# speedinghzl/DSRG

Hardware: AMD Instinct MI355X
Metric: images/sec DSRG train step (VGG16 321x321, 21-class) (higher is better)
Workload: dtype bf16 backbone (fp32 master weights) + f32/f64 supervision path

## Files before the change

dsrg_amd/_lib.py:

```python
import ctypes
import os

import torch

_HERE = os.path.dirname(os.path.abspath(__file__))
LIB_PATH = os.path.join(_HERE, os.environ.get("DSRG_LIB") or "libdsrg_hip.so")

OK, ERR_INVALID, ERR_HIP, ERR_UNSUPPORTED, ERR_NOMEM = 0, -1, -2, -3, -4


class DsrgError(RuntimeError):
    def __init__(self, code, msg):
        RuntimeError.__init__(self, "libdsrg_hip error %d: %s" % (code, msg))
        self.code = code


class CrfParams(ctypes.Structure):
    _fields_ = [("w_bilateral", ctypes.c_float), ("theta_alpha_x", ctypes.c_float),
                ("theta_alpha_y", ctypes.c_float), ("theta_beta_r", ctypes.c_float),
                ("theta_beta_g", ctypes.c_float), ("theta_beta_b", ctypes.c_float),
                ("w_gaussian", ctypes.c_float), ("theta_gamma_x", ctypes.c_float),
                ("theta_gamma_y", ctypes.c_float), ("n_iters", ctypes.c_int32)]

    @classmethod
# ... 46 lines not shown
    "dsrg_seed_loss_plain": (_i, [_i, _i, _i, _vp, _vp, _vp, _vp, _vp]),
    "dsrg_expand_loss": (_i, [_i, _i, _i, _vp, _vp, _d, _d, _vp, _vp, _vp, _vp]),
    "dsrg_confusion_matrix": (_i, [_sz, _vp, _vp, _i, _i, _vp, _vp]),
    "dsrg_multiscale_unary": (_i, [_i, _i, ctypes.POINTER(_vp), ctypes.POINTER(ctypes.c_int32), ctypes.POINTER(ctypes.c_int32), _i, _i,
                                   _f, _vp, _vp, _vp, _vp]),
    "dsrg_im2col3x3_nhwc16": (_i, [_vp, _vp, _i, _i, _i, _i, _i, _vp]),
    "dsrg_relu_bwd_bias_bf16": (_i, [_vp, _vp, _vp, _vp, _vp, _i, ctypes.c_long, _i, ctypes.c_float, _vp]),
    "dsrg_col2im3x3_nhwc_bf16": (_i, [_vp, _vp, _i, _i, _i, _i, _i, _vp]),
    "dsrg_avgpool3x3_s1_bf16": (_i, [_vp, _vp, _i, _i, _i, _i, _vp]),
    "dsrg_conv_igemm_backward_residual_bf16": (_i, [_vp] * 8 + [_i, _vp, _sz] + [_i] * 6 + [_vp]),
    "dsrg_pack_conv_weight_scaled_f32": (_i, [_vp, _vp, _vp, _vp, _i, _i, _i, _vp]),
    "dsrg_aspp_shift_sum_f32": (_i, [_vp, _vp, _vp, _vp] + [_i] * 6 + [_vp]),
    "dsrg_aspp_shift_gather_bf16": (_i, [_vp, _vp, _vp] + [_i] * 6 + [_vp]),
    "dsrg_defer_reductions": (_i, [_i]),
    "dsrg_flush_reductions": (_i, [_vp]),
    "dsrg_conv_igemm_residual_bf16": (_i, [_vp] * 6 + [_i] * 8 + [_vp]),
    "dsrg_conv_igemm_split_f32": (_i, [_vp, _vp, _vp, _vp] + [_i] * 8 + [_vp]),
    "dsrg_add_relu_bf16": (_i, [_vp, _vp, _vp, _sz, _vp]),
    "dsrg_relu_mask_bf16": (_i, [_vp, _vp, _vp, _vp, _sz, _vp]),
    "dsrg_bias_grad_bf16": (_i, [_vp, _vp, _vp, _i, ctypes.c_long, _i, _vp]),
    "dsrg_heads_forward_bf16": (_i, [_vp, _i, _vp, _vp, _vp, _i, _i, _i, _i, _vp]),
    "dsrg_conv3x3_direct_bf16": (_i, [_vp, _vp, _vp, _vp, _i, _i, _i, _i, _i, _i, _vp]),
    "dsrg_conv3x3_direct_dgrad_workspace": (_sz, [_i]),
    "dsrg_conv3x3_direct_dgrad_bf16": (_i, [_vp] * 6 + [_sz] + [_i] * 5 + [_vp]),
    "dsrg_conv_igemm_supported": (_i, [_i, _i, _i]),
    "dsrg_conv_igemm_bf16": (_i, [_vp, _vp, _vp, _vp, _vp, _i, _i, _i, _i, _i, _i, _i, _i, ctypes.c_float, ctypes.c_ulonglong, _vp, _sz,
                                  _vp]),
    "dsrg_conv_igemm_workspace": (_sz, []),
    "dsrg_conv_igemm_dgrad_workspace": (_sz, [_i] * 5),
    "dsrg_conv_igemm_dgrad_bf16": (_i, [_vp] * 6 + [_i] * 7 + [_f, _vp, _sz, _vp]),
# ... 51 lines not shown
```

dsrg_amd/csrc/backbone_ops.hip:

```cpp
#include "common.h"
#include <algorithm>
#include <cstring>

namespace dsrg {

__device__ __forceinline__ float bf16_lo(uint32_t w) { return __uint_as_float(w << 16); }
__device__ __forceinline__ float bf16_hi(uint32_t w) { return __uint_as_float(w & 0xffff0000u); }
__device__ __forceinline__ uint32_t f32_to_bf16_rne(float f) {
    uint32_t u = __float_as_uint(f);
    if ((u & 0x7fffffffu) > 0x7f800000u) return (u >> 16) | 0x40u;
    return (u + 0x7fffu + ((u >> 16) & 1u)) >> 16;
}
__device__ __forceinline__ uint32_t pack_bf16(float lo, float hi) { return f32_to_bf16_rne(lo) | (f32_to_bf16_rne(hi) << 16); }

constexpr int kRbThreads = 256;

__global__ __launch_bounds__(kRbThreads) void relu_bwd_bias_kernel(const uint4 *__restrict__ g, const uint4 *__restrict__ y,
                                                                    uint4 *__restrict__ gm, float *__restrict__ part,
                                                                    int rows, int C8, int rows_per_block, float scale) {
    __shared__ float red[kRbThreads][9];
    const int lanes_r = kRbThreads / C8;
    const int cg = threadIdx.x % C8, rl = threadIdx.x / C8;
    float acc[8] = {0.f, 0.f, 0.f, 0.f, 0.f, 0.f, 0.f, 0.f};
    if (rl < lanes_r) {
// ... 1066 lines not shown
    if (gw) {
        HeadArgs a;
        for (int k = 0; k < 4; k++) a.x[k] = static_cast<const uint16_t *>(x[k < nbr ? k : 0]);
        a.w = w; a.bias = nullptr; a.out = nullptr; a.nbr = nbr; a.M = M; a.K = K; a.O = O; a.HW = HW;
        const int nch = heads_bwd_chunks(M), rows = ((M + nch - 1) / nch + 1) & ~1;
        const size_t lds = (size_t)kDwRows2 * (K * 2 + 64) + 32 * kDwGPitch * sizeof(float);
        if (lds > 160 * 1024) {
            hipLaunchKernelGGL(heads_bwd_dw_kernel, dim3(nch, nbr), dim3(256), 0, stream, a, g, partial, rows);
        } else {
            static LdsGrant grant;
            if (int rc2 = ensure_dynamic_lds(reinterpret_cast<const void *>(&heads_bwd_dw_split_kernel), lds, grant)) return rc2;
            hipLaunchKernelGGL(heads_bwd_dw_split_kernel, dim3(nch, nbr), dim3(256), lds, stream, a, g, partial, rows);
        }
        DSRG_LAUNCH_CHECK();
        const size_t n = (size_t)nbr * O * K;
        hipLaunchKernelGGL(heads_bwd_dw_reduce_kernel, dim3((unsigned)((n + 255) / 256)), dim3(256), 0, stream, partial, gw, nch, n);
        DSRG_LAUNCH_CHECK();
    }
    return DSRG_OK;
}

}
```

dsrg_amd/csrc/common.h:

```cpp
#pragma once
#include <hip/hip_runtime.h>
#include <stdint.h>
#include <stddef.h>
#include <atomic>
#include "../../include/dsrg_hip.h"

namespace dsrg {

int set_error(int code, const char *fmt, ...);
#define DSRG_HIP_CHECK(expr)                                                              \
    do {                                                                                  \
        hipError_t _e = (expr);                                                           \
        if (_e != hipSuccess)                                                             \
            return ::dsrg::set_error(DSRG_ERR_HIP, "%s failed: %s (%s:%d)", #expr,        \
                                     hipGetErrorString(_e), __FILE__, __LINE__);          \
    } while (0)
#define DSRG_LAUNCH_CHECK() DSRG_HIP_CHECK(hipGetLastError())

__device__ __forceinline__ void colsum_block(const float *__restrict__ p, float *__restrict__ out, int rows, int cout, int bx, float (*red)[64]) {
    const int cl = threadIdx.x & 63, c = bx * 64 + cl, q = threadIdx.x >> 6;
    float s0 = 0.0f, s1 = 0.0f;
    int r = q;
    for (; r + 16 < rows; r += 32) {
        s0 += p[(size_t)r * cout + c];
// ... 23 lines not shown
            s2 += part[(size_t)(b + 16) * C + c];
            s3 += part[(size_t)(b + 24) * C + c];
        }
        for (; b < nblk; b += 8) s0 += part[(size_t)b * C + c];
    }
    if (on) red[sl][cl] = (s0 + s1) + (s2 + s3);
    __syncthreads();
    if (on && sl == 0 && c < C) {
        float s = 0.f;
#pragma unroll
        for (int k = 0; k < 8; ++k) s += red[k][cl];
        bias_grad[c] = s;
    }
}
bool defer_reduction(int kind, const float *part, float *out, int rows, int cols);

struct LdsGrant { std::atomic<size_t> bytes[16]; LdsGrant() { for (auto &b : bytes) b.store(0, std::memory_order_relaxed); } };
inline int ensure_dynamic_lds(const void *fn, size_t bytes, std::atomic<size_t> &granted) {
    size_t have = granted.load(std::memory_order_acquire);
    if (bytes <= have) return DSRG_OK;
    if (bytes > 64 * 1024) {
        hipError_t e = hipFuncSetAttribute(fn, hipFuncAttributeMaxDynamicSharedMemorySize, (int)bytes);
        if (e != hipSuccess)
            return set_error(DSRG_ERR_HIP, "cannot reserve %zu B of dynamic LDS: %s", bytes, hipGetErrorString(e));
    }
    while (have < bytes && !granted.compare_exchange_weak(have, bytes, std::memory_order_release, std::memory_order_acquire)) {}
    return DSRG_OK;
}
inline int ensure_dynamic_lds(const void *fn, size_t bytes, LdsGrant &g) {
    int dev = 0;
// ... 200 lines not shown
```

dsrg_amd/csrc/conv_direct.hip:

```cpp
#include "common.h"

namespace dsrg {
namespace {
typedef __attribute__((ext_vector_type(8))) __bf16 bf16x8;
typedef __attribute__((ext_vector_type(2))) __bf16 bf16x2;
typedef __attribute__((ext_vector_type(2))) float f32x2;
typedef __attribute__((ext_vector_type(16))) float f32x16;
typedef __attribute__((address_space(3))) void lds_void;
constexpr int kTH = 8, kTW = 16;
constexpr int kHH = kTH + 2, kHW = kTW + 2;

template <int CIN, int COUT, int TPW_ = (CIN == 64 ? 2 : 1)> struct Cfg {
    static constexpr int CG = CIN / 16;
    static constexpr int KS = 9 * CG;
    static constexpr int TPW = TPW_;
    static constexpr int WGS = TPW * KS * 4 <= 144 ? 2 : 1;
    static constexpr int NG = COUT / (32 * TPW);
    static constexpr int PG = 4 / NG;
    static constexpr int MT = 4 / PG;
    static constexpr int KPS = WGS == 2 ? 2 : 4;
    static constexpr int SPT = CG / KPS;
    static constexpr int STEPS = 9 * SPT;
    static constexpr bool DMA = CIN == 128 && COUT == 128;
    static constexpr int CPR = CIN / 8;
// ... 751 lines not shown
    a.B = B; a.H = H; a.W = W; a.cin = cin; a.roles = cin < 64 ? 1 : cin / 64;
    a.tiles_x = (W + kTW - 1) / kTW; a.tiles_y = (H + kTH - 1) / kTH;
    const long items = (long)B * a.tiles_x * a.tiles_y * a.roles;
    if (B < 1 || H < 1 || W < 1 || items > 0x7fffffffL) return set_error(DSRG_ERR_INVALID, "conv3x3_wgrad: bad shape");
    a.nitems = (int)items;
    const int grid = wgrad_grid(B, H, W, cin, cout);
    if (workspace_bytes < conv3x3_wgrad_workspace(B, H, W, cin, cout))
        return set_error(DSRG_ERR_INVALID, "conv3x3_wgrad: workspace of %zu bytes, %zu needed", workspace_bytes,
                         conv3x3_wgrad_workspace(B, H, W, cin, cout));
    if (cin == 3) {
        static LdsGrant grant;
        const size_t lds = 2 * kHH * kHW * kC3Pix + 3 * kTH * kTW * kC3Row;
        if (int rc = ensure_dynamic_lds(reinterpret_cast<const void *>(&conv3x3_c3_wgrad_kernel), lds, grant)) return rc;
        hipLaunchKernelGGL(conv3x3_c3_wgrad_kernel, dim3(grid), dim3(256), lds, stream, a);
        DSRG_LAUNCH_CHECK();
        if (out_f32) hipLaunchKernelGGL(conv3x3_c3_wgrad_reduce_kernel<true>, dim3(64), dim3(1024), 0, stream, workspace, gw, grid);
        else hipLaunchKernelGGL(conv3x3_c3_wgrad_reduce_kernel<false>, dim3(64), dim3(1024), 0, stream, workspace, gw, grid);
        DSRG_LAUNCH_CHECK();
        return DSRG_OK;
    }
    if (int rc = cout == 64 ? launch_wgrad_variant<2>(a, grid, stream) : launch_wgrad_variant<4>(a, grid, stream)) return rc;
    if (out_f32)
        hipLaunchKernelGGL(conv3x3_wgrad_reduce_kernel<true>, dim3(cout * 9 * cin / 64), dim3(1024), 0, stream, workspace, gw, grid, a.roles,
                           cout, cin);
    else
        hipLaunchKernelGGL(conv3x3_wgrad_reduce_kernel<false>, dim3(cout * 9 * cin / 64), dim3(1024), 0, stream, workspace, gw, grid, a.roles,
                           cout, cin);
    DSRG_LAUNCH_CHECK();
    return DSRG_OK;
}

bool conv3x3_direct_supported(int cin, int cout) {
    return ((cin == 64 || cin == 128) && (cout == 64 || cout == 128)) || (cin == 3 && cout == 64);
}

size_t conv3x3_direct_colsum_workspace(int cout) { return (size_t)2 * device_cus() * (size_t)cout * sizeof(float); }

int launch_conv3x3_direct(const void *x, const void *w, const float *bias, void *y, int B, int H, int W, int cin, int cout,
                          int relu, hipStream_t stream, const void *mask, float *colsum, void *colsum_ws, size_t colsum_ws_bytes) {
    if (!conv3x3_direct_supported(cin, cout))
        return set_error(DSRG_ERR_INVALID, "conv3x3_direct: %d -> %d channels is not one of 64/128 -> 64/128 or 3 -> 64", cin, cout);
    if ((mask || colsum) && (cin == 3 || !mask || !colsum))
        return set_error(DSRG_ERR_UNSUPPORTED, "conv3x3_direct: the masked form takes 64 / 128 channels, mask and bias gradient together");
    if (mask && (long long)B * H * W * cout * 2 >= 0x7fffffffLL)
// ... 30 lines not shown
```

dsrg_amd/csrc/conv_igemm.hip:

```cpp
#include "common.h"
#include <algorithm>
#include <cstdlib>
#include <cstring>
#include <functional>
#include <map>
#include <mutex>
#include <queue>
#include <vector>

namespace dsrg {
namespace {
typedef __attribute__((ext_vector_type(8))) __bf16 bf16x8;
typedef __attribute__((ext_vector_type(2))) __bf16 bf16x2;
typedef __attribute__((ext_vector_type(2))) float f32x2;
typedef __attribute__((ext_vector_type(16))) float f32x16;
typedef __attribute__((address_space(3))) void lds_void;

constexpr int kBM = 256, kBN = 256;
constexpr int kOutRow = 128 * 2 + 16;
constexpr int kOutWave = 64 * kOutRow;
constexpr uint32_t kOob = 0x80000000u;
constexpr int kRowTab = 8 * kOutWave;
constexpr int kRowTabBytes = kBM * 4;

// ... 1369 lines not shown
    const int ks_mix = wgrad_ksplit(M, tiles, 256, (double)ngroups * cout * k * k * cin * 4.0, true);
    if (ks_mix > ks) ks = ks_mix;
    if (ngroups == 1) ks = wgrad_ksplit_cap(M, ks);
    return (size_t)ngroups * ks * cout * k * k * cin * sizeof(float);
}

static int launch_wgrad_reduce(const IgemmWgradArgs &a, void *const *gw, int ngroups, int cin, int cout, int k, int out_bf16, hipStream_t stream) {
    WgradReduceArgs r;
    memset(&r, 0, sizeof(r));
    r.ksplit = a.ksplit;
    r.n4 = (size_t)cout * k * k * cin / 4;
    r.scale = t_wgrad_scale;
    r.per_o4 = (size_t)k * k * cin / 4;
    for (int q = 0; q < ngroups; q++) { r.part[q] = a.g[q].part; r.gw[q] = gw[q]; }
    const dim3 rgrid((unsigned)((r.n4 + 255) / 256), (unsigned)ngroups);
    if (out_bf16) hipLaunchKernelGGL(conv_igemm_wgrad_reduce_kernel<true>, rgrid, dim3(256), 0, stream, r);
    else hipLaunchKernelGGL(conv_igemm_wgrad_reduce_kernel<false>, rgrid, dim3(256), 0, stream, r);
    DSRG_LAUNCH_CHECK();
    return DSRG_OK;
}

int launch_conv_igemm_wgrad(const void *const *x, const void *const *g, void *const *gw, const int *dil, int ngroups, void *workspace,
                            size_t workspace_bytes, int B, int H, int W, int cin, int cout, int k, int out_bf16, hipStream_t stream) {
    if (ngroups < 1 || ngroups > 4) return set_error(DSRG_ERR_INVALID, "conv_igemm_wgrad: 1..4 groups");
    if (!conv_igemm_wgrad_launchable(cin, cout, k))
        return set_error(DSRG_ERR_UNSUPPORTED, "conv_igemm_wgrad: cin %% 64 == 0, cout %% 64 == 0, k in (1, 3) required (got %d, %d, %d)", cin, cout, k);
    const long long M = (long long)B * H * W;
    if (M <= 0 || M * cin * 2 >= 0x7fffffffLL || M * cout * 2 >= 0x7fffffffLL)
        return set_error(DSRG_ERR_UNSUPPORTED, "conv_igemm_wgrad: tensor too large for 32-bit buffer offsets");
    const size_t need = conv_igemm_wgrad_workspace(ngroups, B, H, W, cin, cout, k);
    if (!workspace || workspace_bytes < need) return set_error(DSRG_ERR_INVALID, "conv_igemm_wgrad: workspace of %zu bytes needed", need);
    IgemmWgradArgs a;
    memset(&a, 0, sizeof(a));
    a.ngroups = ngroups; a.B = B; a.H = H; a.W = W; a.Cin = cin; a.Cout = cout; a.taps = k * k; a.M = (int)M;
// ... 170 lines not shown
```

dsrg_amd/csrc/deferred.hip:

```cpp
#include "common.h"
#include <mutex>
#include <cstring>

namespace dsrg {
namespace {

constexpr int kMaxDeferred = 48;
struct DeferredReduction {
    const float *part;
    float *out;
    int rows, cols, kind, first_block;
};
struct DeferredArgs {
    DeferredReduction e[kMaxDeferred];
    int n;
};

__global__ __launch_bounds__(1024) void deferred_reductions_kernel(DeferredArgs a) {
    __shared__ float red_c[16][64];
    __shared__ float red_b[8][33];
    const int b = (int)blockIdx.x;
    int k = 0;
    while (k + 1 < a.n && b >= a.e[k + 1].first_block) k++;
    const DeferredReduction d = a.e[k];
    if (d.kind == 0) colsum_block(d.part, d.out, d.rows, d.cols, b - d.first_block, red_c);
    else bias_finalize_block(d.part, d.out, d.rows, d.cols, b - d.first_block, red_b);
}

std::mutex g_mutex;
bool g_on = false;
DeferredArgs g_list;
int g_blocks = 0;

}

bool defer_reduction(int kind, const float *part, float *out, int rows, int cols) {
    std::lock_guard<std::mutex> lock(g_mutex);
    if (!g_on || g_list.n >= kMaxDeferred || rows < 1 || cols < 1 || (kind == 0 && cols % 64)) return false;
    DeferredReduction &d = g_list.e[g_list.n++];
    d.part = part; d.out = out; d.rows = rows; d.cols = cols; d.kind = kind; d.first_block = g_blocks;
    g_blocks += kind == 0 ? cols / 64 : (cols + 31) / 32;
    return true;
}

int defer_reductions(int on) {
    std::lock_guard<std::mutex> lock(g_mutex);
    if (on && !g_on) { memset(&g_list, 0, sizeof(g_list)); g_blocks = 0; }
    g_on = on != 0;
    return DSRG_OK;
}

int flush_reductions(hipStream_t stream) {
    DeferredArgs a;
    int blocks;
    {
        std::lock_guard<std::mutex> lock(g_mutex);
        a = g_list;
        blocks = g_blocks;
        memset(&g_list, 0, sizeof(g_list));
        g_blocks = 0;
    }
    if (a.n == 0) return DSRG_OK;
    hipLaunchKernelGGL(deferred_reductions_kernel, dim3(blocks), dim3(1024), 0, stream, a);
    DSRG_LAUNCH_CHECK();
    return DSRG_OK;
}

}

extern "C" int dsrg_defer_reductions(int on) { return dsrg::defer_reductions(on); }
extern "C" int dsrg_flush_reductions(void *stream) { return dsrg::flush_reductions(static_cast<hipStream_t>(stream)); }
```

dsrg_amd/ops.py:

```python
import ctypes
import threading

import torch

from . import _lib
from ._lib import CrfParams, check


def _stream():
    return ctypes.c_void_p(torch.cuda.current_stream().cuda_stream)


def _ptr(t):
    return ctypes.c_void_p(t.data_ptr()) if t is not None else None


def _f32c(t, name):
    if not (t.is_cuda and t.dtype == torch.float32 and t.is_contiguous()):
        raise ValueError("%s must be a contiguous float32 CUDA tensor" % name)
    return t


_defer = [False]
_defer_keep = []


def _keep_until_flush(*tensors):
    if _defer[0]:
        _defer_keep.extend(t for t in tensors if t is not None)


@__import__("contextlib").contextmanager
def deferred_reductions(enabled=True):
    if not enabled or _defer[0]:
        yield
        return
    L = _lib.lib()
    check(L.dsrg_defer_reductions(1))
    _defer[0] = True
    try:
        yield
    finally:
        _defer[0] = False
        rc = L.dsrg_flush_reductions(_stream())
        L.dsrg_defer_reductions(0)
        del _defer_keep[:]
        check(rc)


class Context(object):

    def __init__(self, max_batch, C, H, W):
        _lib.require_gpu()
        self.max_batch, self.C, self.H, self.W = int(max_batch), int(C), int(H), int(W)
        self.device = torch.cuda.current_device()
        h = ctypes.c_void_p()
        check(_lib.lib().dsrg_ctx_create(self.max_batch, self.C, self.H, self.W, ctypes.byref(h)))
        self._h = h
# ... 597 lines not shown
    else:
        _check_kept_packs(weight, fwd, dg, pack)
    return fwd, (dg if want_dgrad else None)


def conv3x3_wgrad(x, g, out_dtype=torch.bfloat16, out=None):
    B, cin, H, W = x.shape
    cout = g.shape[1]
    cl = torch.channels_last
    if not (x.is_cuda and x.dtype == torch.bfloat16 and g.dtype == torch.bfloat16 and tuple(g.shape) == (B, cout, H, W)
            and (cin, cout) in WGRAD_CONV_SHAPES):
        raise ValueError("conv3x3_wgrad needs bf16 CUDA tensors with (cin, cout) in %s" % (WGRAD_CONV_SHAPES,))
    x = x if x.is_contiguous(memory_format=cl) else x.contiguous(memory_format=cl)
    g = g if g.is_contiguous(memory_format=cl) else g.contiguous(memory_format=cl)
    need = _lib.lib().dsrg_conv3x3_wgrad_workspace(B, H, W, cin, cout)
    key = (x.device.index, torch.cuda.current_stream().cuda_stream)
    ws = _wgrad_ws.get(key)
    if ws is None or ws.numel() < need:
        ws = _wgrad_ws[key] = torch.empty(need, dtype=torch.uint8, device=x.device)
    if out_dtype not in (torch.bfloat16, torch.float32):
        raise ValueError("conv3x3_wgrad: bf16 or float32 output")
    gw = _dest(out, (cout, cin, 3, 3), out_dtype, x.device, True)
    fn = _lib.lib().dsrg_conv3x3_wgrad_f32 if out_dtype == torch.float32 else _lib.lib().dsrg_conv3x3_wgrad_bf16
    check(fn(_ptr(x), _ptr(g), _ptr(gw), _ptr(ws), ws.numel(), B, H, W, cin, cout, _stream()))
    return gw


def conv_igemm_supported(cin, cout, k):
    return bool(_lib.lib().dsrg_conv_igemm_supported(int(cin), int(cout), int(k)))


def set_igemm_variant(v):
    _lib.lib().dsrg_debug_set_igemm_variant(int(v))


def pack_conv_weight(weight, for_dgrad=False, dtype=torch.bfloat16):
    k = weight.shape[2]
# ... 148 lines not shown

def conv_igemm_backward(g, packed_d, x, dilation, mask=None, mask_scale=1.0, ksize=3, gw_out=None, gb_out=None):
    B, cout, H, W = g.shape
    cin = x.shape[1]
    cl = torch.channels_last
    if not (g.is_cuda and g.dtype == torch.bfloat16 and x.dtype == torch.bfloat16 and tuple(x.shape) == (B, cin, H, W)
            and packed_d.dtype == torch.bfloat16 and tuple(packed_d.shape) == (cin, cout // 64, ksize * ksize, 64)
            and packed_d.is_contiguous() and x.is_contiguous(memory_format=cl)
            and (mask is None or (mask.dtype == torch.bfloat16 and tuple(mask.shape) == (B, cin, H, W) and mask.is_contiguous(memory_format=cl)))):
        raise ValueError("conv_igemm_backward needs bf16 channels_last g / x (/ mask) of one geometry and the data-gradient packing")
    g = g if g.is_contiguous(memory_format=cl) else g.contiguous(memory_format=cl)
    L = _lib.lib()
    need = L.dsrg_conv_igemm_wgrad_workspace(1, B, H, W, cin, cout, ksize)
    if need == 0:
        raise ValueError("conv_igemm_backward: 256 | cin (or cin = 128), 256 | cout required (got %d, %d)" % (cin, cout))
    key = (g.device.index, torch.cuda.current_stream().cuda_stream)
    ws = _igemm_ws.get(key)
    if ws is None or ws.numel() < need:
        ws = _igemm_ws[key] = torch.empty(need, dtype=torch.uint8, device=g.device)
    gx = torch.empty((B, cin, H, W), dtype=torch.bfloat16, device=g.device, memory_format=cl)
    gw = _dest(gw_out, (cout, cin, ksize, ksize), torch.float32, g.device, True)
    gb = cws = None
    if mask is not None:
        gb = _dest(gb_out, (cin,), torch.float32, g.device)
        cws = torch.empty(L.dsrg_conv_igemm_dgrad_workspace(1, B, H, W, cin), dtype=torch.uint8, device=g.device)
        _keep_until_flush(cws)
    check(L.dsrg_conv_igemm_backward_bf16(_ptr(g), _ptr(packed_d), _ptr(x), _ptr(mask), _ptr(gx), _ptr(gw), int(dilation), _ptr(gb),
                                          float(mask_scale), _ptr(cws), cws.numel() if cws is not None else 0, _ptr(ws), ws.numel(),
                                          B, H, W, cin, cout, ksize, _stream()))
    return gx, gw, gb


def conv_igemm_backward_residual(g, packed_d, x, dilation, ksize, mask=None, res=None, gw_scale=None, gw_out=None):
    B, cout, H, W = g.shape
    cin = x.shape[1]
    cl = torch.channels_last
    ok = lambda t: t.dtype == torch.bfloat16 and tuple(t.shape) == (B, cin, H, W) and t.is_contiguous(memory_format=cl)
    if not (g.is_cuda and g.dtype == torch.bfloat16 and ok(x) and packed_d.dtype == torch.bfloat16 and packed_d.is_contiguous()
            and tuple(packed_d.shape) == (cin, cout // 64, ksize * ksize, 64) and (mask is None or ok(mask)) and (res is None or ok(res))):
        raise ValueError("conv_igemm_backward_residual needs bf16 channels_last g / x (/ mask / res) of one geometry and the data-gradient packing")
    g = g if g.is_contiguous(memory_format=cl) else g.contiguous(memory_format=cl)
    L = _lib.lib()
    need = L.dsrg_conv_igemm_wgrad_workspace(1, B, H, W, cin, cout, ksize)
    if need == 0:
        raise ValueError("conv_igemm_backward_residual: 256 | cin (or cin = 128 with a 3x3 kernel), 256 | cout required (got %d, %d)" % (cin, cout))
    key = (g.device.index, torch.cuda.current_stream().cuda_stream)
    ws = _igemm_ws.get(key)
    if ws is None or ws.numel() < need:
        ws = _igemm_ws[key] = torch.empty(need, dtype=torch.uint8, device=g.device)
    gx = torch.empty((B, cin, H, W), dtype=torch.bfloat16, device=g.device, memory_format=cl)
    gw = _dest(gw_out, (cout, cin, ksize, ksize), torch.float32, g.device, True)
    sc = None if gw_scale is None else _f32c(gw_scale, "gw_scale")
    check(L.dsrg_conv_igemm_backward_residual_bf16(_ptr(g), _ptr(packed_d), _ptr(x), _ptr(mask), _ptr(res), _ptr(gx), _ptr(gw), _ptr(sc),
                                                   int(dilation), _ptr(ws), ws.numel(), B, H, W, cin, cout, ksize, _stream()))
    return gx, gw


_igemm_sk_ws = {}


def _igemm_sk_workspace(device):
    key = (device.index, torch.cuda.current_stream(device).cuda_stream)
    ws = _igemm_sk_ws.get(key)
    if ws is None:
        ws = _igemm_sk_ws[key] = torch.empty(_lib.lib().dsrg_conv_igemm_workspace(), dtype=torch.uint8, device=device)
    return ws

# ... 27 lines not shown
    B, cin, H, W = xs[0].shape
    cout = gs[0].shape[1]
    cl = torch.channels_last
    if not (1 <= n <= 4 and len(gs) == n and len(dilations) == n) or out_dtype not in (torch.float32, torch.bfloat16):
        raise ValueError("conv_igemm_wgrad: 1..4 groups, float32 or bfloat16 result")
    for x, g in zip(xs, gs):
        if not (x.is_cuda and x.dtype == torch.bfloat16 and g.dtype == torch.bfloat16 and tuple(x.shape) == (B, cin, H, W)
                and tuple(g.shape) == (B, cout, H, W)):
            raise ValueError("conv_igemm_wgrad needs bf16 CUDA tensors of one geometry")
    xs = [x if x.is_contiguous(memory_format=cl) else x.contiguous(memory_format=cl) for x in xs]
    gs = [g if g.is_contiguous(memory_format=cl) else g.contiguous(memory_format=cl) for g in gs]
    L = _lib.lib()
    need = L.dsrg_conv_igemm_wgrad_workspace(n, B, H, W, cin, cout, ksize)
    if need == 0:
        raise ValueError("conv_igemm_wgrad: 64 | cin, 64 | cout, k in (1, 3) required (got %d, %d, %d)" % (cin, cout, ksize))
    key = (xs[0].device.index, torch.cuda.current_stream().cuda_stream)
    ws = _igemm_ws.get(key)
    if ws is None or ws.numel() < need:
        ws = _igemm_ws[key] = torch.empty(need, dtype=torch.uint8, device=xs[0].device)
    gws = [_dest(outs[i] if outs is not None else None, (cout, cin, ksize, ksize), out_dtype, xs[0].device, True) for i in range(n)]
    vp = ctypes.c_void_p * n
    check(L.dsrg_conv_igemm_wgrad_bf16(vp(*[x.data_ptr() for x in xs]), vp(*[g.data_ptr() for g in gs]),
                                       vp(*[w.data_ptr() for w in gws]), (ctypes.c_int * n)(*[int(d) for d in dilations]), n,
                                       _ptr(ws), ws.numel(), B, H, W, cin, cout, ksize, int(out_dtype == torch.bfloat16), _stream()))
    return gws


def heads_forward(xs, weight, bias):
    B, K, H, W = xs[0].shape
    n, O = weight.shape[0], weight.shape[1]
    cl = torch.channels_last
    xs = [x if x.is_contiguous(memory_format=cl) else x.contiguous(memory_format=cl) for x in xs]
    if not all(x.is_cuda and x.dtype == torch.bfloat16 and x.shape == xs[0].shape for x in xs) or len(xs) != n:
        raise ValueError("heads_forward needs n bf16 CUDA activations of one shape")
    _f32c(weight, "weight")
# ... 6 lines not shown


def heads_backward(xs, weight, g, need_gx=True, relu_scale=0.0):
    B, K, H, W = xs[0].shape
    n, O = weight.shape[0], weight.shape[1]
    cl = torch.channels_last
    xs = [x if x.is_contiguous(memory_format=cl) else x.contiguous(memory_format=cl) for x in xs]
    _f32c(weight, "weight")
    g = g.contiguous()
    _f32c(g, "g")
    L = _lib.lib()
    M = B * H * W
    gx = torch.empty((n, B, H, W, K), dtype=torch.bfloat16, device=g.device) if need_gx else None
    gw = torch.empty((n, O, K), dtype=torch.float32, device=g.device)
    part = torch.empty(L.dsrg_heads_backward_chunks(M) * n * O * K, dtype=torch.float32, device=g.device)
    ptrs = (ctypes.c_void_p * 4)(*([x.data_ptr() for x in xs] + [None] * (4 - n)))
    if relu_scale > 0.0 and need_gx:
        gb = torch.empty((n, K), dtype=torch.float32, device=g.device)
        ws = torch.empty(L.dsrg_heads_backward_relu_workspace(n, M, K), dtype=torch.uint8, device=g.device)
        _keep_until_flush(ws)
        check(L.dsrg_heads_backward_relu_bf16(ptrs, n, _ptr(weight), _ptr(g), _ptr(gx), M * K * 2, _ptr(gw), _ptr(part),
                                              float(relu_scale), _ptr(gb), _ptr(ws), ws.numel(), B, H * W, K, O, _stream()))
        return [gx[k].permute(0, 3, 1, 2) for k in range(n)], gw, gb
    check(L.dsrg_heads_backward_bf16(ptrs, n, _ptr(weight), _ptr(g), _ptr(gx), M * K * 2, _ptr(gw), _ptr(part), B, H * W, K, O,
                                     _stream()))
    return ([gx[k].permute(0, 3, 1, 2) for k in range(n)] if need_gx else None), gw


def maxpool3x3_out_size(n, stride, ceil_mode):
    num = n + 2 - 3
    o = (-(-num // stride) if ceil_mode else num // stride) + 1
    if (o - 1) * stride >= n + 1:
        o -= 1
# ... 59 lines not shown
```

dsrg_amd/retrain.py:

```python
import torch
import torch.nn as nn
import torch.nn.functional as F

import os as _os

from .backbone import VGG16ASPP, GemmConv2d, _ConvFn, _bf16_run
from .trainer import CaffeSGD

_FUSE_RES = _os.environ.get("DSRG_RESNET_FUSE_RES", "1") == "1"


def interp_shrink(label, factor=8):
    H, W = label.shape[-2:]
    if (H - 1) % factor == 0 and (W - 1) % factor == 0:
        return label[..., ::factor, ::factor]
    h, w = (H - 1) // factor + 1, (W - 1) // factor + 1
    return F.interpolate(label.float(), size=(h, w), mode="bilinear", align_corners=True)


def seg_softmax_loss(logits, label, ignore_label=255):
    return F.cross_entropy(logits.float(), label.reshape(label.shape[0], *label.shape[-2:]).long(),
                           ignore_index=ignore_label, reduction="mean")


# ... 341 lines not shown
    def load(self, state_path):
        from .checkpoint import load_snapshot
        return load_snapshot(self, state_path)

    def step(self, images, label):
        if self.reducer is not None:
            self.reducer.prepare()
        else:
            self.opt.zero_grad()
        self.opt.base_lr = poly_lr(self.base_lr, self.opt.iter, self.max_iter)
        x = images.contiguous(memory_format=torch.channels_last) if self.device.type == "cuda" else images
        with torch.autocast(self.device.type, dtype=self.amp_dtype, enabled=self.amp_dtype is not None):
            logits = self.net(x)
        loss = seg_softmax_loss(logits, interp_shrink(label, 8))
        from .ops import deferred_reductions
        with deferred_reductions(self.defer_bias):
            loss.backward()
        if self.reducer is not None:
            self.reducer.finish()
        self.opt.step()
        return loss.detach()
```

dsrg_amd/trainer.py:

```python
import os

import torch

from .backbone import VGG16ASPP
from .ops import dsrg_supervision_loss


_SGD_PACK = os.environ.get("DSRG_SGD_PACK", "1") != "0"


class CaffeSGD(object):

    def __init__(self, groups, base_lr=5e-4, momentum=0.9, weight_decay=5e-4, gamma=0.33, stepsize=1000):
        self.groups = groups
        self.base_lr, self.momentum, self.wd, self.gamma, self.stepsize = base_lr, momentum, weight_decay, gamma, stepsize
        self.iter = 0
        for g in self.groups:
            g["bufs"] = [torch.zeros_like(p, memory_format=torch.preserve_format) for p in g["params"]]
            g["buf_lr"] = None
        if _SGD_PACK:
            from .ops import keep_weight_packs
            keep_weight_packs([p for g in self.groups for p in g["params"] if p.is_cuda], self)

    def lr(self):
# ... 155 lines not shown
        if self.overlap_build:
            from .ops import crf_prepare
            main = torch.cuda.current_stream()
            self.side.wait_stream(main)
            with torch.cuda.stream(self.side):
                crf_prepare(images, cues.shape[1], cues.shape[2], cues.shape[3])
        with torch.autocast(self.device.type, dtype=self.amp_dtype, enabled=self.amp_dtype is not None):
            logits = self.net(x)
        logits = logits.float().contiguous()
        if self.overlap_build:
            torch.cuda.current_stream().wait_stream(self.side)
            total, losses = self.loss_fn(logits, images, labels, cues, prepared=True)
        else:
            total, losses = self.loss_fn(logits, images, labels, cues)
        from .ops import deferred_reductions
        with deferred_reductions(self.defer_bias):
            total.backward()
        if self.reducer is not None:
            self.reducer.finish()
        self.opt.step()
        return losses
```

include/dsrg_hip.h:

```cpp
#ifndef DSRG_HIP_H
#define DSRG_HIP_H

#include <stddef.h>
#include <stdint.h>

#ifdef __cplusplus
extern "C" {
#endif

#pragma GCC visibility push(default)

#define DSRG_OK 0
#define DSRG_ERR_INVALID (-1)
#define DSRG_ERR_HIP (-2)
#define DSRG_ERR_UNSUPPORTED (-3)
#define DSRG_ERR_NOMEM (-4)

const char *dsrg_last_error(void);
int dsrg_device_count(void);
int dsrg_host_register(void *host, size_t bytes);
int dsrg_host_unregister(void *host);

typedef struct dsrg_crf_s *dsrg_crf_t;

// ... 113 lines not shown
                         float dropout_p, unsigned long long dropout_seed, void *workspace_dev, size_t workspace_bytes,
                         void *stream);
size_t dsrg_conv_igemm_workspace(void);
size_t dsrg_conv_igemm_dgrad_workspace(int ngroups, int B, int H, int W, int cout);
int dsrg_conv_igemm_dgrad_bf16(const void *const *g_dev, const void *const *w_dev, const void *const *mask_dev, void *const *gx_dev,
                               float *const *bias_grad_dev, const int *dilation, int ngroups, int B, int H, int W, int cin,
                               int cout, int ksize, float mask_scale, void *workspace_dev, size_t workspace_bytes, void *stream);
int dsrg_conv_igemm_residual_bf16(const void *x_dev, const void *w_dev, const float *bias_dev, const void *res_dev, const void *mask_dev,
                                  void *y_dev, int dilation, int B, int H, int W, int cin, int cout, int ksize, int relu, void *stream);
int dsrg_aspp_shift_sum_f32(const void *y_dev, const float *bias_dev, float *out_dev, const int *offsets, int npairs, int outputs,
                            int channels, int B, int H, int W, void *stream);
int dsrg_aspp_shift_gather_bf16(const float *g_dev, void *gp_dev, const int *offsets, int npairs, int outputs, int channels, int B, int H,
                                int W, void *stream);
int dsrg_defer_reductions(int on);
int dsrg_flush_reductions(void *stream);
int dsrg_conv_igemm_workspace_status(const void *workspace_dev, void *stream, int *status_host);
int dsrg_pack_conv_weight_f32(const float *w_dev, void *fwd_dev, void *dgrad_dev, int cout, int cin, int ksize, void *stream);
int dsrg_pack_conv_weight_scaled_f32(const float *w_dev, const float *scale_dev, void *fwd_dev, void *dgrad_dev, int cout, int cin,
                                     int ksize, void *stream);
int dsrg_sgd_pack_f32(int n, float *const *param_dev, const float *const *grad_dev, float *const *momentum_dev, void *const *fwd_dev,
                      void *const *dgrad_dev, const int *shape, const long long *numel, const float *lr, const float *weight_decay,
                      float momentum, void *stream);
size_t dsrg_conv_igemm_wgrad_workspace(int ngroups, int B, int H, int W, int cin, int cout, int ksize);
int dsrg_conv_igemm_wgrad_bf16(const void *const *x_dev, const void *const *g_dev, void *const *gw_dev, const int *dilation,
                               int ngroups, void *workspace_dev, size_t workspace_bytes, int B, int H, int W, int cin, int cout,
                               int ksize, int out_bf16, void *stream);
int dsrg_conv_igemm_backward_bf16(const void *g_dev, const void *w_dgrad_dev, const void *x_dev, const void *mask_dev, void *gx_dev,
                                  float *gw_dev, int dilation, float *bias_grad_dev, float mask_scale, void *colsum_workspace_dev,
                                  size_t colsum_workspace_bytes, void *wgrad_workspace_dev, size_t wgrad_workspace_bytes, int B, int H,
                                  int W, int cin, int cout, int ksize, void *stream);
// ... 38 lines not shown
```

Measured before the change: 1941.

## Run weight-gradient reduction kernels on a low-priority side stream during backward

Weight-gradient reduce kernels (direct conv, igemm wgrad, heads dW) are no longer launched inline on the main stream. Inside the deferred-reductions scope they are queued and forked in batches onto a per-device low-priority side stream, ordered by events, and the main stream waits on a tail event at flush. The goal is to overlap these reductions with the rest of the backward pass. In exchange, wgrad scratch buffers are allocated per call instead of reused from a cache, more tensors are kept alive until flush, and event and host overhead grows. The path is disabled when a gradient reducer is present or when the stream is being captured.

```diff
diff --git a/dsrg_amd/_lib.py b/dsrg_amd/_lib.py
--- a/dsrg_amd/_lib.py
+++ b/dsrg_amd/_lib.py
@@ -84,6 +84,7 @@
     "dsrg_aspp_shift_gather_bf16": (_i, [_vp, _vp, _vp] + [_i] * 6 + [_vp]),
     "dsrg_defer_reductions": (_i, [_i]),
     "dsrg_flush_reductions": (_i, [_vp]),
+    "dsrg_reductions_outstanding": (_i, []),
     "dsrg_conv_igemm_residual_bf16": (_i, [_vp] * 6 + [_i] * 8 + [_vp]),
     "dsrg_conv_igemm_split_f32": (_i, [_vp, _vp, _vp, _vp] + [_i] * 8 + [_vp]),
     "dsrg_add_relu_bf16": (_i, [_vp, _vp, _vp, _sz, _vp]),
diff --git a/dsrg_amd/csrc/backbone_ops.hip b/dsrg_amd/csrc/backbone_ops.hip
--- a/dsrg_amd/csrc/backbone_ops.hip
+++ b/dsrg_amd/csrc/backbone_ops.hip
@@ -1104,10 +1104,11 @@
         }
         DSRG_LAUNCH_CHECK();
         const size_t n = (size_t)nbr * O * K;
-        hipLaunchKernelGGL(heads_bwd_dw_reduce_kernel, dim3((unsigned)((n + 255) / 256)), dim3(256), 0, stream, partial, gw, nch, n);
-        DSRG_LAUNCH_CHECK();
-    }
-    return DSRG_OK;
-}
-
-}
+        if (int rc2 = launch_reduction(stream, [=](hipStream_t s) {
+                hipLaunchKernelGGL(heads_bwd_dw_reduce_kernel, dim3((unsigned)((n + 255) / 256)), dim3(256), 0, s, partial, gw, nch, n);
+            })) return rc2;
+    }
+    return DSRG_OK;
+}
+
+}
diff --git a/dsrg_amd/csrc/common.h b/dsrg_amd/csrc/common.h
--- a/dsrg_amd/csrc/common.h
+++ b/dsrg_amd/csrc/common.h
@@ -3,6 +3,7 @@
 #include <stdint.h>
 #include <stddef.h>
 #include <atomic>
+#include <functional>
 #include "../../include/dsrg_hip.h"
 
 namespace dsrg {
@@ -61,6 +62,7 @@
     }
 }
 bool defer_reduction(int kind, const float *part, float *out, int rows, int cols);
+int launch_reduction(hipStream_t stream, const std::function<void(hipStream_t)> &launch);
 
 struct LdsGrant { std::atomic<size_t> bytes[16]; LdsGrant() { for (auto &b : bytes) b.store(0, std::memory_order_relaxed); } };
 inline int ensure_dynamic_lds(const void *fn, size_t bytes, std::atomic<size_t> &granted) {
diff --git a/dsrg_amd/csrc/conv_direct.hip b/dsrg_amd/csrc/conv_direct.hip
--- a/dsrg_amd/csrc/conv_direct.hip
+++ b/dsrg_amd/csrc/conv_direct.hip
@@ -789,20 +789,21 @@
         if (int rc = ensure_dynamic_lds(reinterpret_cast<const void *>(&conv3x3_c3_wgrad_kernel), lds, grant)) return rc;
         hipLaunchKernelGGL(conv3x3_c3_wgrad_kernel, dim3(grid), dim3(256), lds, stream, a);
         DSRG_LAUNCH_CHECK();
-        if (out_f32) hipLaunchKernelGGL(conv3x3_c3_wgrad_reduce_kernel<true>, dim3(64), dim3(1024), 0, stream, workspace, gw, grid);
-        else hipLaunchKernelGGL(conv3x3_c3_wgrad_reduce_kernel<false>, dim3(64), dim3(1024), 0, stream, workspace, gw, grid);
-        DSRG_LAUNCH_CHECK();
-        return DSRG_OK;
+        return launch_reduction(stream, [=](hipStream_t s) {
+            if (out_f32) hipLaunchKernelGGL(conv3x3_c3_wgrad_reduce_kernel<true>, dim3(64), dim3(1024), 0, s, workspace, gw, grid);
+            else hipLaunchKernelGGL(conv3x3_c3_wgrad_reduce_kernel<false>, dim3(64), dim3(1024), 0, s, workspace, gw, grid);
+        });
     }
     if (int rc = cout == 64 ? launch_wgrad_variant<2>(a, grid, stream) : launch_wgrad_variant<4>(a, grid, stream)) return rc;
-    if (out_f32)
-        hipLaunchKernelGGL(conv3x3_wgrad_reduce_kernel<true>, dim3(cout * 9 * cin / 64), dim3(1024), 0, stream, workspace, gw, grid, a.roles,
-                           cout, cin);
-    else
-        hipLaunchKernelGGL(conv3x3_wgrad_reduce_kernel<false>, dim3(cout * 9 * cin / 64), dim3(1024), 0, stream, workspace, gw, grid, a.roles,
-                           cout, cin);
-    DSRG_LAUNCH_CHECK();
-    return DSRG_OK;
+    const int roles = a.roles;
+    return launch_reduction(stream, [=](hipStream_t s) {
+        if (out_f32)
+            hipLaunchKernelGGL(conv3x3_wgrad_reduce_kernel<true>, dim3(cout * 9 * cin / 64), dim3(1024), 0, s, workspace, gw, grid, roles, cout,
+                               cin);
+        else
+            hipLaunchKernelGGL(conv3x3_wgrad_reduce_kernel<false>, dim3(cout * 9 * cin / 64), dim3(1024), 0, s, workspace, gw, grid, roles, cout,
+                               cin);
+    });
 }
 
 bool conv3x3_direct_supported(int cin, int cout) {
diff --git a/dsrg_amd/csrc/conv_igemm.hip b/dsrg_amd/csrc/conv_igemm.hip
--- a/dsrg_amd/csrc/conv_igemm.hip
+++ b/dsrg_amd/csrc/conv_igemm.hip
@@ -1407,10 +1407,10 @@
     r.per_o4 = (size_t)k * k * cin / 4;
     for (int q = 0; q < ngroups; q++) { r.part[q] = a.g[q].part; r.gw[q] = gw[q]; }
     const dim3 rgrid((unsigned)((r.n4 + 255) / 256), (unsigned)ngroups);
-    if (out_bf16) hipLaunchKernelGGL(conv_igemm_wgrad_reduce_kernel<true>, rgrid, dim3(256), 0, stream, r);
-    else hipLaunchKernelGGL(conv_igemm_wgrad_reduce_kernel<false>, rgrid, dim3(256), 0, stream, r);
-    DSRG_LAUNCH_CHECK();
-    return DSRG_OK;
+    return launch_reduction(stream, [=](hipStream_t s) {
+        if (out_bf16) hipLaunchKernelGGL(conv_igemm_wgrad_reduce_kernel<true>, rgrid, dim3(256), 0, s, r);
+        else hipLaunchKernelGGL(conv_igemm_wgrad_reduce_kernel<false>, rgrid, dim3(256), 0, s, r);
+    });
 }
 
 int launch_conv_igemm_wgrad(const void *const *x, const void *const *g, void *const *gw, const int *dil, int ngroups, void *workspace,
diff --git a/dsrg_amd/csrc/deferred.hip b/dsrg_amd/csrc/deferred.hip
--- a/dsrg_amd/csrc/deferred.hip
+++ b/dsrg_amd/csrc/deferred.hip
@@ -1,6 +1,7 @@
 #include "common.h"
 #include <mutex>
 #include <cstring>
+#include <vector>
 
 namespace dsrg {
 namespace {
@@ -29,9 +30,94 @@
 
 std::mutex g_mutex;
 bool g_on = false;
+bool g_side_on = false;
 DeferredArgs g_list;
 int g_blocks = 0;
 
+constexpr int kSideBatch = 4;
+constexpr bool kSideLowPriority = true;
+constexpr int kSideEvents = 16;
+constexpr int kMaxDevices = 16;
+struct SideStream {
+    hipStream_t stream = nullptr;
+    hipEvent_t fork[kSideEvents] = {}, tail = nullptr;
+    int forks = 0;
+    int running = 0;
+    hipStream_t owner = nullptr;
+    std::vector<std::function<void(hipStream_t)>> pending;
+};
+SideStream g_side[kMaxDevices];
+
+int side_create(SideStream &s) {
+    if (s.stream) return DSRG_OK;
+    hipStream_t st = nullptr;
+    if (kSideLowPriority) {
+        int least = 0, greatest = 0;
+        DSRG_HIP_CHECK(hipDeviceGetStreamPriorityRange(&least, &greatest));
+        DSRG_HIP_CHECK(hipStreamCreateWithPriority(&st, hipStreamNonBlocking, least));
+    } else {
+        DSRG_HIP_CHECK(hipStreamCreateWithFlags(&st, hipStreamNonBlocking));
+    }
+    for (int k = 0; k < kSideEvents; k++) DSRG_HIP_CHECK(hipEventCreateWithFlags(&s.fork[k], hipEventDisableTiming));
+    DSRG_HIP_CHECK(hipEventCreateWithFlags(&s.tail, hipEventDisableTiming));
+    s.stream = st;
+    return DSRG_OK;
+}
+
+int side_fork(SideStream &s) {
+    if (s.pending.empty()) return DSRG_OK;
+    hipStream_t where = s.owner;
+    if (s.forks < kSideEvents) {
+        if (int rc = side_create(s)) return rc;
+        hipEvent_t ev = s.fork[s.forks++];
+        DSRG_HIP_CHECK(hipEventRecord(ev, s.owner));
+        DSRG_HIP_CHECK(hipStreamWaitEvent(s.stream, ev, 0));
+        where = s.stream;
+        s.running += (int)s.pending.size();
+    }
+    for (auto &launch : s.pending) launch(where);
+    s.pending.clear();
+    DSRG_LAUNCH_CHECK();
+    return DSRG_OK;
+}
+
+int side_drain(SideStream &s) {
+    for (auto &launch : s.pending) launch(s.owner);
+    const bool any = !s.pending.empty();
+    s.pending.clear();
+    if (any) DSRG_LAUNCH_CHECK();
+    return DSRG_OK;
+}
+
+}
+
+int launch_reduction(hipStream_t stream, const std::function<void(hipStream_t)> &launch) {
+    std::lock_guard<std::mutex> lock(g_mutex);
+    int dev = 0;
+    bool side = g_on && g_side_on && hipGetDevice(&dev) == hipSuccess && dev >= 0 && dev < kMaxDevices;
+    if (side) {
+        hipStreamCaptureStatus cap = hipStreamCaptureStatusNone;
+        if (hipStreamIsCapturing(stream, &cap) != hipSuccess) { (void)hipGetLastError(); cap = hipStreamCaptureStatusActive; }
+        side = cap == hipStreamCaptureStatusNone;
+    }
+    if (!side) {
+        launch(stream);
+        DSRG_LAUNCH_CHECK();
+        return DSRG_OK;
+    }
+    SideStream &s = g_side[dev];
+    if (!s.pending.empty() && s.owner != stream)
+        if (int rc = side_fork(s)) return rc;
+    s.owner = stream;
+    s.pending.push_back(launch);
+    return (int)s.pending.size() >= kSideBatch ? side_fork(s) : DSRG_OK;
+}
+
+int reductions_outstanding() {
+    std::lock_guard<std::mutex> lock(g_mutex);
+    int n = g_list.n;
+    for (const SideStream &s : g_side) n += s.running + (int)s.pending.size();
+    return n;
 }
 
 bool defer_reduction(int kind, const float *part, float *out, int rows, int cols) {
@@ -47,6 +133,7 @@
     std::lock_guard<std::mutex> lock(g_mutex);
     if (on && !g_on) { memset(&g_list, 0, sizeof(g_list)); g_blocks = 0; }
     g_on = on != 0;
+    g_side_on = g_on && !(on & 2);
     return DSRG_OK;
 }
 
@@ -60,9 +147,21 @@
         memset(&g_list, 0, sizeof(g_list));
         g_blocks = 0;
     }
-    if (a.n == 0) return DSRG_OK;
-    hipLaunchKernelGGL(deferred_reductions_kernel, dim3(blocks), dim3(1024), 0, stream, a);
-    DSRG_LAUNCH_CHECK();
+    if (a.n > 0) {
+        hipLaunchKernelGGL(deferred_reductions_kernel, dim3(blocks), dim3(1024), 0, stream, a);
+        DSRG_LAUNCH_CHECK();
+    }
+    std::lock_guard<std::mutex> lock(g_mutex);
+    int dev = 0;
+    if (hipGetDevice(&dev) != hipSuccess || dev < 0 || dev >= kMaxDevices) { (void)hipGetLastError(); return DSRG_OK; }
+    SideStream &s = g_side[dev];
+    if (int rc = side_drain(s)) return rc;
+    if (s.running > 0) {
+        DSRG_HIP_CHECK(hipEventRecord(s.tail, s.stream));
+        DSRG_HIP_CHECK(hipStreamWaitEvent(stream, s.tail, 0));
+    }
+    s.running = 0;
+    s.forks = 0;
     return DSRG_OK;
 }
 
@@ -70,3 +169,4 @@
 
 extern "C" int dsrg_defer_reductions(int on) { return dsrg::defer_reductions(on); }
 extern "C" int dsrg_flush_reductions(void *stream) { return dsrg::flush_reductions(static_cast<hipStream_t>(stream)); }
+extern "C" int dsrg_reductions_outstanding(void) { return dsrg::reductions_outstanding(); }
diff --git a/dsrg_amd/ops.py b/dsrg_amd/ops.py
--- a/dsrg_amd/ops.py
+++ b/dsrg_amd/ops.py
@@ -22,6 +22,7 @@
 
 
 _defer = [False]
+_side = [False]
 _defer_keep = []
 
 
@@ -30,18 +31,36 @@
         _defer_keep.extend(t for t in tensors if t is not None)
 
 
+def _keep_alias(*tensors):
+    if _defer[0]:
+        _defer_keep.extend(t.detach() for t in tensors if t is not None)
+
+
+def _wgrad_scratch(cache, need, device):
+    if _side[0]:
+        ws = torch.empty(need, dtype=torch.uint8, device=device)
+        _defer_keep.append(ws)
+        return ws
+    key = (device.index, torch.cuda.current_stream().cuda_stream)
+    ws = cache.get(key)
+    if ws is None or ws.numel() < need:
+        ws = cache[key] = torch.empty(need, dtype=torch.uint8, device=device)
+    return ws
+
+
 @__import__("contextlib").contextmanager
-def deferred_reductions(enabled=True):
+def deferred_reductions(enabled=True, weight_grads=True):
     if not enabled or _defer[0]:
         yield
         return
     L = _lib.lib()
-    check(L.dsrg_defer_reductions(1))
+    check(L.dsrg_defer_reductions(1 if weight_grads else 3))
     _defer[0] = True
+    _side[0] = bool(weight_grads)
     try:
         yield
     finally:
-        _defer[0] = False
+        _defer[0] = _side[0] = False
         rc = L.dsrg_flush_reductions(_stream())
         L.dsrg_defer_reductions(0)
         del _defer_keep[:]
@@ -669,13 +688,11 @@
     x = x if x.is_contiguous(memory_format=cl) else x.contiguous(memory_format=cl)
     g = g if g.is_contiguous(memory_format=cl) else g.contiguous(memory_format=cl)
     need = _lib.lib().dsrg_conv3x3_wgrad_workspace(B, H, W, cin, cout)
-    key = (x.device.index, torch.cuda.current_stream().cuda_stream)
-    ws = _wgrad_ws.get(key)
-    if ws is None or ws.numel() < need:
-        ws = _wgrad_ws[key] = torch.empty(need, dtype=torch.uint8, device=x.device)
+    ws = _wgrad_scratch(_wgrad_ws, need, x.device)
     if out_dtype not in (torch.bfloat16, torch.float32):
         raise ValueError("conv3x3_wgrad: bf16 or float32 output")
     gw = _dest(out, (cout, cin, 3, 3), out_dtype, x.device, True)
+    _keep_alias(gw)
     fn = _lib.lib().dsrg_conv3x3_wgrad_f32 if out_dtype == torch.float32 else _lib.lib().dsrg_conv3x3_wgrad_bf16
     check(fn(_ptr(x), _ptr(g), _ptr(gw), _ptr(ws), ws.numel(), B, H, W, cin, cout, _stream()))
     return gw
@@ -854,10 +871,7 @@
     need = L.dsrg_conv_igemm_wgrad_workspace(1, B, H, W, cin, cout, ksize)
     if need == 0:
         raise ValueError("conv_igemm_backward: 256 | cin (or cin = 128), 256 | cout required (got %d, %d)" % (cin, cout))
-    key = (g.device.index, torch.cuda.current_stream().cuda_stream)
-    ws = _igemm_ws.get(key)
-    if ws is None or ws.numel() < need:
-        ws = _igemm_ws[key] = torch.empty(need, dtype=torch.uint8, device=g.device)
+    ws = _wgrad_scratch(_igemm_ws, need, g.device)
     gx = torch.empty((B, cin, H, W), dtype=torch.bfloat16, device=g.device, memory_format=cl)
     gw = _dest(gw_out, (cout, cin, ksize, ksize), torch.float32, g.device, True)
     gb = cws = None
@@ -865,6 +879,7 @@
         gb = _dest(gb_out, (cin,), torch.float32, g.device)
         cws = torch.empty(L.dsrg_conv_igemm_dgrad_workspace(1, B, H, W, cin), dtype=torch.uint8, device=g.device)
         _keep_until_flush(cws)
+    _keep_alias(gw, gb)
     check(L.dsrg_conv_igemm_backward_bf16(_ptr(g), _ptr(packed_d), _ptr(x), _ptr(mask), _ptr(gx), _ptr(gw), int(dilation), _ptr(gb),
                                           float(mask_scale), _ptr(cws), cws.numel() if cws is not None else 0, _ptr(ws), ws.numel(),
                                           B, H, W, cin, cout, ksize, _stream()))
@@ -884,13 +899,11 @@
     need = L.dsrg_conv_igemm_wgrad_workspace(1, B, H, W, cin, cout, ksize)
     if need == 0:
         raise ValueError("conv_igemm_backward_residual: 256 | cin (or cin = 128 with a 3x3 kernel), 256 | cout required (got %d, %d)" % (cin, cout))
-    key = (g.device.index, torch.cuda.current_stream().cuda_stream)
-    ws = _igemm_ws.get(key)
-    if ws is None or ws.numel() < need:
-        ws = _igemm_ws[key] = torch.empty(need, dtype=torch.uint8, device=g.device)
+    ws = _wgrad_scratch(_igemm_ws, need, g.device)
     gx = torch.empty((B, cin, H, W), dtype=torch.bfloat16, device=g.device, memory_format=cl)
     gw = _dest(gw_out, (cout, cin, ksize, ksize), torch.float32, g.device, True)
     sc = None if gw_scale is None else _f32c(gw_scale, "gw_scale")
+    _keep_alias(gw, sc)
     check(L.dsrg_conv_igemm_backward_residual_bf16(_ptr(g), _ptr(packed_d), _ptr(x), _ptr(mask), _ptr(res), _ptr(gx), _ptr(gw), _ptr(sc),
                                                    int(dilation), _ptr(ws), ws.numel(), B, H, W, cin, cout, ksize, _stream()))
     return gx, gw
@@ -948,11 +961,9 @@
     need = L.dsrg_conv_igemm_wgrad_workspace(n, B, H, W, cin, cout, ksize)
     if need == 0:
         raise ValueError("conv_igemm_wgrad: 64 | cin, 64 | cout, k in (1, 3) required (got %d, %d, %d)" % (cin, cout, ksize))
-    key = (xs[0].device.index, torch.cuda.current_stream().cuda_stream)
-    ws = _igemm_ws.get(key)
-    if ws is None or ws.numel() < need:
-        ws = _igemm_ws[key] = torch.empty(need, dtype=torch.uint8, device=xs[0].device)
+    ws = _wgrad_scratch(_igemm_ws, need, xs[0].device)
     gws = [_dest(outs[i] if outs is not None else None, (cout, cin, ksize, ksize), out_dtype, xs[0].device, True) for i in range(n)]
+    _keep_alias(*gws)
     vp = ctypes.c_void_p * n
     check(L.dsrg_conv_igemm_wgrad_bf16(vp(*[x.data_ptr() for x in xs]), vp(*[g.data_ptr() for g in gs]),
                                        vp(*[w.data_ptr() for w in gws]), (ctypes.c_int * n)(*[int(d) for d in dilations]), n,
@@ -989,9 +1000,12 @@
     gx = torch.empty((n, B, H, W, K), dtype=torch.bfloat16, device=g.device) if need_gx else None
     gw = torch.empty((n, O, K), dtype=torch.float32, device=g.device)
     part = torch.empty(L.dsrg_heads_backward_chunks(M) * n * O * K, dtype=torch.float32, device=g.device)
+    _keep_until_flush(part)
+    _keep_alias(gw)
     ptrs = (ctypes.c_void_p * 4)(*([x.data_ptr() for x in xs] + [None] * (4 - n)))
     if relu_scale > 0.0 and need_gx:
         gb = torch.empty((n, K), dtype=torch.float32, device=g.device)
+        _keep_alias(gb)
         ws = torch.empty(L.dsrg_heads_backward_relu_workspace(n, M, K), dtype=torch.uint8, device=g.device)
         _keep_until_flush(ws)
         check(L.dsrg_heads_backward_relu_bf16(ptrs, n, _ptr(weight), _ptr(g), _ptr(gx), M * K * 2, _ptr(gw), _ptr(part),
diff --git a/dsrg_amd/retrain.py b/dsrg_amd/retrain.py
--- a/dsrg_amd/retrain.py
+++ b/dsrg_amd/retrain.py
@@ -379,7 +379,7 @@
             logits = self.net(x)
         loss = seg_softmax_loss(logits, interp_shrink(label, 8))
         from .ops import deferred_reductions
-        with deferred_reductions(self.defer_bias):
+        with deferred_reductions(self.defer_bias, weight_grads=self.reducer is None):
             loss.backward()
         if self.reducer is not None:
             self.reducer.finish()
diff --git a/dsrg_amd/trainer.py b/dsrg_amd/trainer.py
--- a/dsrg_amd/trainer.py
+++ b/dsrg_amd/trainer.py
@@ -193,7 +193,7 @@
         else:
             total, losses = self.loss_fn(logits, images, labels, cues)
         from .ops import deferred_reductions
-        with deferred_reductions(self.defer_bias):
+        with deferred_reductions(self.defer_bias, weight_grads=self.reducer is None):
             total.backward()
         if self.reducer is not None:
             self.reducer.finish()
diff --git a/include/dsrg_hip.h b/include/dsrg_hip.h
--- a/include/dsrg_hip.h
+++ b/include/dsrg_hip.h
@@ -151,6 +151,7 @@
                                 int W, void *stream);
 int dsrg_defer_reductions(int on);
 int dsrg_flush_reductions(void *stream);
+int dsrg_reductions_outstanding(void);
 int dsrg_conv_igemm_workspace_status(const void *workspace_dev, void *stream, int *status_host);
 int dsrg_pack_conv_weight_f32(const float *w_dev, void *fwd_dev, void *dgrad_dev, int cout, int cin, int ksize, void *stream);
 int dsrg_pack_conv_weight_scaled_f32(const float *w_dev, const float *scale_dev, void *fwd_dev, void *dgrad_dev, int cout, int cin,
```

Result: no change. 1948, median of 6 (+0.4%).
